# clevercool/ANT-Quantization

Hardware: AMD Instinct MI355X
Metric: Gelements/s quant-dequant + achieved HBM GB/s %peak, 4-bit ANT, 1/8 MI355X (higher is better)
Workload: dtype f32; 1 GPU; headline: 32 x [4096,4096] bf16 weight tensors per GPU, ANT 4-bit signed flint grid, calibrated per-row alpha, steady-state _forward; one step = ONE batched launch (antq_fakequant_batch) over all 32 tensors; io_dtype=bf16

## Files before the change

ant_quantization_amd/csrc/antq_host.h:

```cpp
#ifndef ANTQ_HOST_H
#define ANTQ_HOST_H

#include <hip/hip_runtime.h>
#include <stdint.h>
#include <string.h>

#include <algorithm>
#include <vector>

#include "../../include/antq.h"
#include "antq_internal.h"
#include "antq_device.h"
#include "antq_k_approx.h"

namespace antq {

extern thread_local int g_knob_u;
extern thread_local int g_knob_encwg;
extern thread_local int g_knob_x;
extern thread_local int g_knob_nearest_fast;
extern thread_local int g_knob_lane_rows;
extern thread_local int g_knob_a;
extern thread_local int g_knob_waves;
extern thread_local int g_knob_rot;
extern thread_local int g_knob_lane_u;
extern thread_local int g_knob_h;
extern thread_local int g_knob_hist;
extern thread_local int g_knob_sweep;
extern thread_local int g_knob_sort_short;
extern thread_local int g_knob_sort;
extern thread_local int g_knob_tk_group, g_knob_tk_blocks;
extern thread_local int g_knob_rows_stream;
extern thread_local int g_knob_hist_xmax;
extern thread_local int g_knob_exp;
extern thread_local int g_knob_schunks;
extern thread_local int g_knob_dlds;
extern thread_local int g_knob_hlds;

static inline bool plan_args_from_host(const void *plan_host, PlanArgs &pa)
{
    const PlanHeader *h = static_cast<const PlanHeader *>(plan_host);
    if (h->magic != kPlanMagic || h->version != kPlanVersion) return false;
    if (h->m < 1 || h->m > ANTQ_MAX_GRID || h->m_pad != ((h->m + 3) & ~3u)) return false;
    pa.kind = h->kind;
    pa.m = h->m;
    pa.m_pad = h->m_pad;
    pa.shift = h->shift;
    pa.kmin = h->kmin;
    pa.kmax = h->kmax;
    pa.keymask = h->keymask;
    pa.nbneg = h->nbneg;
    pa.fastlim = h->fastlim;
    pa.n_entries = (h->kind == kPlanLut) ? h->n_entries : 0;
    pa.tab_units = pa.n_entries + (pa.m_pad >> 2);
    pa.linear = h->linear;
    pa.lin_scale = h->lin_scale;
    pa.lin_bias = h->lin_bias;
    pa.adom = (h->kind == kPlanLut && g_knob_a != 0) ? h->adom : 0u;
    pa.xlim = h->xlim;
    pa.atab_slots = h->atab_slots;
    return true;
}

static inline const uint4 *plan_tab_ptr(const void *plan_dev)
{
    return reinterpret_cast<const uint4 *>(static_cast<const char *>(plan_dev) + sizeof(PlanHeader));
}

static inline size_t lds_table(const PlanArgs &pa, bool idx)
{
    const size_t plain = (size_t)pa.tab_units * 16;
    return pa.adom ? std::max(plain, (size_t)atab_units(pa.atab_slots, pa.m_pad, idx) * 16) : plain;
}

}

#endif
```

ant_quantization_amd/csrc/antq_kernels.hip:

```cpp
#include <type_traits>

#include "antq_host.h"
#include "antq_k_fakequant.h"
#include "antq_k_nearest.h"
#include "antq_k_aux.h"
#include "antq_k_reduce.h"
#include "antq_k_search.h"

namespace antq {

thread_local int g_knob_u = 0;
thread_local int g_knob_encwg = 2048;
thread_local int g_knob_x = 1;
thread_local int g_knob_nearest_fast = 1;
thread_local int g_knob_lane_rows = 1;
thread_local int g_knob_a = 1;
thread_local int g_knob_waves = 0;
thread_local int g_knob_lane_u = 0;
thread_local int g_knob_rot = 0;
thread_local int g_knob_h = 1;
thread_local int g_knob_hlds = -1;
thread_local int g_knob_dlds = -1;
thread_local int g_knob_schunks = 0;
thread_local int g_knob_exp = 0;
thread_local int g_knob_hist = 1;
thread_local int g_knob_hist_xmax = 1;
thread_local int g_knob_rows_stream = 1;
thread_local int g_knob_tk_group = 0;
thread_local int g_knob_tk_blocks = 0;
thread_local int g_knob_sort_short = 1;
thread_local int g_knob_sort = 1;
thread_local int g_knob_sweep = 1;

}

using namespace antq;

extern "C" int antq_abi_version(void) { return ANTQ_ABI_VERSION; }

extern "C" const char *antq_strerror(int code)
{
    switch (code) {
    case ANTQ_OK: return "ok";
    case ANTQ_ERR_ARG: return "invalid argument";
    case ANTQ_ERR_UNSUPPORTED: return "unsupported dtype / size for this entry point";
    case ANTQ_ERR_PLAN: return "malformed or undersized plan blob";
    case ANTQ_ERR_LAUNCH: return "HIP kernel launch failed";
    case ANTQ_ERR_ALIGN: return "pointer not aligned to the element size";
    default: return "unknown antq error";
    }
}

extern "C" int antq_nearest(const void *x, void *z, int16_t *idx, size_t n, const void *grid, int m, int dtype,
                            void *stream)
{
    if (n == 0) return ANTQ_OK;
    if (!x || !z || !grid || m < 1) return ANTQ_ERR_ARG;
    if (m > ANTQ_MAX_GRID) return ANTQ_ERR_UNSUPPORTED;
    hipStream_t st = static_cast<hipStream_t>(stream);
    if (dtype == ANTQ_F32 || dtype == ANTQ_F64) {
        const size_t blocks = (n + 1023) / 1024;
        if (blocks > 0x7fffffffull) return ANTQ_ERR_UNSUPPORTED;
        if (dtype == ANTQ_F32) {
            if (m <= 256 && g_knob_nearest_fast)
                hipLaunchKernelGGL((k_nearest_fast<float>), dim3((unsigned)((n + 2047) / 2048)), dim3(256), 0, st,
                                   static_cast<const float *>(x), static_cast<float *>(z), idx, n,
                                   static_cast<const float *>(grid), m);
            else
                hipLaunchKernelGGL((k_nearest<float>), dim3((unsigned)blocks), dim3(256), 0, st,
                                   static_cast<const float *>(x), static_cast<float *>(z), idx, n,
                                   static_cast<const float *>(grid), m);
        } else {
            if (m <= 256 && g_knob_nearest_fast)
                hipLaunchKernelGGL((k_nearest_fast<double>), dim3((unsigned)((n + 2047) / 2048)), dim3(256), 0, st,
                                   static_cast<const double *>(x), static_cast<double *>(z), idx, n,
                                   static_cast<const double *>(grid), m);
            else
                hipLaunchKernelGGL((k_nearest<double>), dim3((unsigned)blocks), dim3(256), 0, st,
                                   static_cast<const double *>(x), static_cast<double *>(z), idx, n,
                                   static_cast<const double *>(grid), m);
        }
    } else if (dtype == ANTQ_BF16 || dtype == ANTQ_F16) {
        const size_t blocks = (n + 255) / 256;
        if (blocks > 0x7fffffffull) return ANTQ_ERR_UNSUPPORTED;
        if (dtype == ANTQ_BF16)
            hipLaunchKernelGGL((k_nearest16<bf16_tag>), dim3((unsigned)blocks), dim3(256), 0, st, x, z, idx, n,
                               static_cast<const float *>(grid), m);
        else
            hipLaunchKernelGGL((k_nearest16<f16_tag>), dim3((unsigned)blocks), dim3(256), 0, st, x, z, idx, n,
                               static_cast<const float *>(grid), m);
    } else {
        return ANTQ_ERR_ARG;
    }
    return hipGetLastError() == hipSuccess ? ANTQ_OK : ANTQ_ERR_LAUNCH;
}

static int launch_nearest_plan(const void *x, void *z, int16_t *idx, size_t n, const void *plan_host, const void *plan_dev,
                               const float *gcheck, int m_check, int *stale, int dtype, void *stream)
{
    if (n == 0) return ANTQ_OK;
    if (!x || !z || !plan_host || !plan_dev) return ANTQ_ERR_ARG;
    PlanArgs pa;
    if (!plan_args_from_host(plan_host, pa)) return ANTQ_ERR_PLAN;
    if (gcheck && (uint32_t)m_check != pa.m) return ANTQ_ERR_ARG;
    const int epl = dtype == ANTQ_F32 ? 4 : (dtype == ANTQ_BF16 || dtype == ANTQ_F16) ? 8 : 0;
    if (!epl) return ANTQ_ERR_UNSUPPORTED;
    if (n % epl || reinterpret_cast<uintptr_t>(x) % 16 || reinterpret_cast<uintptr_t>(z) % 16 ||
        (idx && reinterpret_cast<uintptr_t>(idx) % 16))
        return ANTQ_ERR_UNSUPPORTED;
    const size_t n_vec = n / epl;
    hipStream_t st = static_cast<hipStream_t>(stream);
    const size_t lds = (size_t)pa.tab_units * 16;
    const bool u2 = !gcheck && lds <= 2048;
// ... 33 lines not shown
{
    if (!grid_dev || m < 1) return ANTQ_ERR_ARG;
    return launch_nearest_plan(x, z, idx, n, plan_host, plan_dev, grid_dev, m, stale, dtype, stream);
}

extern "C" int antq_affine(const float *x, float *out, int32_t *q, size_t rows, size_t row_len, int k,
                           const float *xmin, const float *xmax, int per_row, void *stream)
{
    if (rows == 0 || row_len == 0) return ANTQ_OK;
    if (!x || !out || !xmin || !xmax || k < 1 || k > 24) return ANTQ_ERR_ARG;
    const size_t n = rows * row_len;
    hipStream_t st = static_cast<hipStream_t>(stream);
    const bool vec = (per_row ? row_len : n) % 4 == 0 && reinterpret_cast<uintptr_t>(x) % 16 == 0 &&
                     reinterpret_cast<uintptr_t>(out) % 16 == 0 && (!q || reinterpret_cast<uintptr_t>(q) % 16 == 0);
    if (vec) {
        const size_t n_vec = n / 4, vpr = (per_row ? row_len : n) / 4;
        const size_t blocks = (n_vec + 256 * kAffineU - 1) / (256 * kAffineU);
        if (blocks > 0x7fffffffull) return ANTQ_ERR_UNSUPPORTED;
        hipLaunchKernelGGL(k_affine_vec, dim3((unsigned)blocks), dim3(256), 0, st, reinterpret_cast<const uint4 *>(x),
                           reinterpret_cast<uint4 *>(out), reinterpret_cast<int4 *>(q), n_vec, vpr, k, xmin, xmax,
                           per_row ? 1 : 0);
        return hipGetLastError() == hipSuccess ? ANTQ_OK : ANTQ_ERR_LAUNCH;
    }
    const size_t blocks = (n + 255) / 256;
    if (blocks > 0x7fffffffull) return ANTQ_ERR_UNSUPPORTED;
    hipLaunchKernelGGL(k_affine, dim3((unsigned)blocks), dim3(256), 0, st, x, out, q, n,
                       row_len, k, xmin, xmax, per_row ? 1 : 0);
    return hipGetLastError() == hipSuccess ? ANTQ_OK : ANTQ_ERR_LAUNCH;
}

extern "C" int antq_copy(const void *src, void *dst, size_t bytes, void *stream)
{
    if (bytes == 0) return ANTQ_OK;
    if (!src || !dst || bytes % 16 || reinterpret_cast<uintptr_t>(src) % 16 || reinterpret_cast<uintptr_t>(dst) % 16)
        return ANTQ_ERR_ARG;
    const size_t n_vec = bytes / 16;
    const size_t blocks = (n_vec + 1023) / 1024;
    if (blocks > 0x7fffffffull) return ANTQ_ERR_UNSUPPORTED;
    hipLaunchKernelGGL(k_copy, dim3((unsigned)blocks), dim3(256), 0, static_cast<hipStream_t>(stream),
                       static_cast<const uint4 *>(src), static_cast<uint4 *>(dst), n_vec);
    return hipGetLastError() == hipSuccess ? ANTQ_OK : ANTQ_ERR_LAUNCH;
}

namespace antq {
int prefetch_unit_fq();
int prefetch_unit_batch();
int prefetch_unit_search();
}
extern "C" int antq_prefetch_kernels(void)
{
    hipFuncAttributes at;
    int rc = hipFuncGetAttributes(&at, reinterpret_cast<const void *>(&k_copy)) == hipSuccess ? ANTQ_OK : ANTQ_ERR_LAUNCH;
    if (antq::prefetch_unit_fq() != ANTQ_OK) rc = ANTQ_ERR_LAUNCH;
    if (antq::prefetch_unit_batch() != ANTQ_OK) rc = ANTQ_ERR_LAUNCH;
    if (antq::prefetch_unit_search() != ANTQ_OK) rc = ANTQ_ERR_LAUNCH;
    (void)hipGetLastError();
    return rc;
}

extern "C" int antq_debug_set(int key, int value)
{
    if (key == 0) g_knob_u = value;
    else if (key == 1) g_knob_encwg = value > 0 ? value : 2048;
    else if (key == 2) g_knob_x = value;
    else if (key == 3) g_knob_nearest_fast = value;
    else if (key == 4) g_knob_a = value;
    else if (key == 5) g_knob_lane_rows = value;
    else if (key == 6) g_knob_waves = value;
    else if (key == 7) g_knob_lane_u = value;
    else if (key == 8) g_knob_rot = value;
    else if (key == 9) g_knob_h = value;
    else if (key == 10) g_knob_hlds = value;
    else if (key == 11) g_knob_dlds = value;
    else if (key == 12) g_knob_schunks = value;
    else if (key == 13) g_knob_exp = value;
    else if (key == 14) g_knob_hist = value;
    else if (key == 15) g_knob_hist_xmax = value;
    else if (key == 16) g_knob_rows_stream = value;
    else if (key == 17) g_knob_tk_group = value;
    else if (key == 18) g_knob_tk_blocks = value;
    else if (key == 19) g_knob_sweep = value;
    else if (key == 20) g_knob_sort = value;
    else if (key == 21) g_knob_sort_short = value;
    else return ANTQ_ERR_ARG;
    return ANTQ_OK;
}

namespace antq {

template <typename T>
static int launch_absmax(const void *x, float *amax, size_t rows, size_t row_len, int per_row, hipStream_t st, bool zero = true)
{
    constexpr int EPL = IO<T>::EPL;
    const bool al = reinterpret_cast<uintptr_t>(x) % 16 == 0;
    const int vec_ok = per_row ? (al && row_len % EPL == 0) : al;
    if (per_row && vec_ok) {
        const size_t vpr = row_len / EPL;
        if (vpr <= 64 && (vpr & (vpr - 1)) == 0) {
            int vshift = 0;
            while (((size_t)1 << vshift) < vpr) vshift++;
            const size_t n_vec = rows * vpr, gblocks = (n_vec + 1023) / 1024;
            if (gblocks > 0x7fffffffull) return ANTQ_ERR_UNSUPPORTED;
            hipLaunchKernelGGL((k_absmax_groups<T>), dim3((unsigned)gblocks), dim3(256), 0, st, static_cast<const uint4 *>(x), amax,
                               n_vec, (uint32_t)vpr, vshift);
            return hipGetLastError() == hipSuccess ? ANTQ_OK : ANTQ_ERR_LAUNCH;
        }
    }
    if (per_row && vec_ok && g_knob_rows_stream && rows <= 0x7fffffffull) {
        const size_t vpr = row_len / EPL;
        const dim3 g((unsigned)(rows < 262144u ? rows : 262144u)), b(64);
        const uint4 *xv = static_cast<const uint4 *>(x);
        bool done = true;
        if (vpr == 128) hipLaunchKernelGGL((k_absmax_rows<T, 2>), g, b, 0, st, xv, amax, (uint32_t)rows);
        else if (vpr == 256) hipLaunchKernelGGL((k_absmax_rows<T, 4>), g, b, 0, st, xv, amax, (uint32_t)rows);
        else if (vpr == 512) hipLaunchKernelGGL((k_absmax_rows<T, 8>), g, b, 0, st, xv, amax, (uint32_t)rows);
        else if (vpr == 1024) hipLaunchKernelGGL((k_absmax_rows<T, 16>), g, b, 0, st, xv, amax, (uint32_t)rows);
        else done = false;
        if (done) return hipGetLastError() == hipSuccess ? ANTQ_OK : ANTQ_ERR_LAUNCH;
    }
    size_t waves = per_row ? rows : (rows * row_len + 64 * EPL * 4 - 1) / (64 * EPL * 4);
    size_t blocks = (waves + 3) / 4;
    if (blocks > (per_row ? 4096u : 256u)) blocks = per_row ? 4096 : 256;
    if (blocks < 1) blocks = 1;
    if (!per_row && zero) hipLaunchKernelGGL(k_zero_f32, dim3(1), dim3(64), 0, st, amax);
    hipLaunchKernelGGL((k_absmax<T>), dim3((unsigned)blocks), dim3(256), 0, st, x, amax, rows, row_len, per_row, vec_ok);
    return hipGetLastError() == hipSuccess ? ANTQ_OK : ANTQ_ERR_LAUNCH;
}
}

namespace antq {
template <typename T>
static int launch_alpha_grad(const void *x, const void *out, const void *gout, double *gsum, double *ws, size_t rows,
                             size_t row_len, int per_row, hipStream_t st)
{
    static_assert(kPartialStride == kPtCand, "k_sum_partials reads partials kPtCand doubles apart");
    constexpr int EPL = IO<T>::EPL;
    const bool al = (reinterpret_cast<uintptr_t>(x) | reinterpret_cast<uintptr_t>(out) | reinterpret_cast<uintptr_t>(gout)) % 16 == 0;
    const int vec_ok = per_row ? (al && row_len % EPL == 0) : al;
    size_t waves = per_row ? rows : (rows * row_len + 64 * EPL * 2 - 1) / (64 * EPL * 2);
    size_t blocks = (waves + 3) / 4;
    const size_t cap = per_row ? 4096 : 1024;
    if (blocks > cap) blocks = cap;
    if (blocks < 1) blocks = 1;
    hipLaunchKernelGGL((k_alpha_grad<T>), dim3((unsigned)blocks), dim3(256), 0, st, x, out, gout, gsum, ws, rows, row_len,
                       per_row, vec_ok);
    if (!per_row) hipLaunchKernelGGL(k_sum_partials, dim3(1), dim3(256), 0, st, ws, (uint32_t)blocks, 1, gsum);
    return hipGetLastError() == hipSuccess ? ANTQ_OK : ANTQ_ERR_LAUNCH;
}
}

extern "C" int antq_alpha_grad(const void *x, const void *out, const void *gout, size_t rows, size_t row_len, int per_row,
                               double *gsum, void *workspace, int dtype, void *stream)
{
    if (rows == 0 || row_len == 0) return ANTQ_OK;
    if (!x || !out || !gout || !gsum || (!per_row && !workspace)) return ANTQ_ERR_ARG;
    double *ws = static_cast<double *>(workspace);
    hipStream_t st = static_cast<hipStream_t>(stream);
    switch (dtype) {
    case ANTQ_F32: return launch_alpha_grad<float>(x, out, gout, gsum, ws, rows, row_len, per_row ? 1 : 0, st);
    case ANTQ_BF16: return launch_alpha_grad<bf16_tag>(x, out, gout, gsum, ws, rows, row_len, per_row ? 1 : 0, st);
    case ANTQ_F16: return launch_alpha_grad<f16_tag>(x, out, gout, gsum, ws, rows, row_len, per_row ? 1 : 0, st);
    default: return ANTQ_ERR_UNSUPPORTED;
    }
}

namespace antq {
// ... 197 lines not shown
```

ant_quantization_amd/csrc/antq_search.hip:

```cpp
#include <cstdio>
#include <cstdlib>
#include <mutex>
#include <vector>

#include "antq_host.h"
#include "antq_k_fakequant.h"
#include "antq_k_search.h"
#include "antq_k_hist.h"
#include "antq_k_sweep.h"
#include "antq_k_sortsearch.h"

#include <type_traits>

namespace antq {

constexpr unsigned kSearchMinVpr = 64;

template <typename T>
static bool hist_eligible(size_t n, bool ovp, const void *x, int nflat)
{
    if constexpr (std::is_same<T, float>::value) return false;
    if (g_knob_hist == 0 || (ovp && g_knob_hist == 3) || n % 8 != 0 || n >= ((size_t)1 << 31) || reinterpret_cast<uintptr_t>(x) % 16 != 0) return false;
    if (g_knob_hist == 2) return true;
    if (ovp) return n >= ((size_t)1 << 20) && (double)n * (double)nflat >= 1.5e8;
    return n >= ((size_t)1 << 19);
}
static bool hist_outlier_bound(const void *plan_host, float gmax, float &bound)
{
    const PlanHeader *h = static_cast<const PlanHeader *>(plan_host);
    if (h->kind != kPlanLut || !h->hdom || !(gmax > 0.0f)) return false;
    const HThr *tl = plan_tlist(plan_host);
    float tmin = INFINITY;
    for (uint32_t i = 0; i < h->h_nthr; i++) {
        const bool lo_out = (tl[i].flags & 1u) != 0u, hi_out = (tl[i].flags & 2u) != 0u;
        if (lo_out != hi_out) tmin = std::min(tmin, fabsf(tl[i].T));
    }
    if (!(tmin < INFINITY)) tmin = 3.0e38f;
    bound = tmin / gmax * 0.999f;
    return true;
}
struct HistXmax {
    float *out = nullptr;
    bool taken = false;
};

template <typename T>
static int launch_hist_search(const void *x, size_t n, const float *xmax, const float *ratios, int ncand, const HistTypes &ht,
                              double *sse, void *ws, bool pairs, float tmin_over_gmax, const int **run_if, hipStream_t st,
                              HistXmax *hx = nullptr)
{
    if constexpr (std::is_same<T, float>::value) {
        return ANTQ_ERR_UNSUPPORTED;
    } else {
        const size_t nv = n / 8;
        uint32_t G = (uint32_t)std::min<size_t>(std::max<size_t>(n / 65536, 16), (size_t)kHistMaxG);
        G = (G + 7u) & ~7u;
        char *w = static_cast<char *>(ws);
        uint32_t *slabs = reinterpret_cast<uint32_t *>(w);
        uint32_t *count = reinterpret_cast<uint32_t *>(w + kHistCountOff);
        HistPairs hp;
        hp.xmax = xmax; hp.ratios = ratios; hp.ncand = ncand; hp.tmin_over_gmax = tmin_over_gmax;
        hp.seg = reinterpret_cast<uint32_t *>(w + kHistSegOff);
        hp.seg_count = reinterpret_cast<uint32_t *>(w + kHistSegCountOff);
        hp.flags = reinterpret_cast<int *>(w + kHistFlagsOff);
        hp.list = reinterpret_cast<uint32_t *>(w + kHistListOff);
        const unsigned nflat = (unsigned)(ht.ntypes * ncand);
        size_t lds = 0;
        for (int t = 0; t < ht.ntypes; t++) lds = std::max(lds, (size_t)ht.pa[t].tab_units * 16);
        if (pairs) {
            hipLaunchKernelGGL(k_hist_clear_flags, dim3(1), dim3(64), 0, st, hp.flags);
            hipLaunchKernelGGL((k_hist16<T, true>), dim3(2 * G), dim3(1024), 0, st, static_cast<const uint4 *>(x), nv, G, slabs, hp, nullptr);
            hipLaunchKernelGGL((k_hist_reduce<true>), dim3(256), dim3(256), 0, st, slabs, G, count, hp, G * 16u);
            hipLaunchKernelGGL((k_hist_score<T, true>), dim3(nflat), dim3(1024), lds, st, count, xmax, ratios, ncand, ht, sse, hp);
            *run_if = hp.flags;
        } else {
            float *const xo = (hx && !hx->taken) ? hx->out : nullptr;
            if (hx && xo) hx->taken = true;
            if (xo)
                hipLaunchKernelGGL((k_hist16<T, false, true>), dim3(2 * G), dim3(1024), 0, st, static_cast<const uint4 *>(x), nv, G, slabs, hp, xo);
            else
                hipLaunchKernelGGL((k_hist16<T, false>), dim3(2 * G), dim3(1024), 0, st, static_cast<const uint4 *>(x), nv, G, slabs, hp, nullptr);
            hipLaunchKernelGGL((k_hist_reduce<false>), dim3(256), dim3(256), 0, st, slabs, G, count, hp, 0u);
            hipLaunchKernelGGL((k_hist_score<T, false>), dim3(nflat), dim3(1024), lds, st, count, xmax, ratios, ncand, ht, sse, hp);
        }
        return hipGetLastError() == hipSuccess ? ANTQ_OK : ANTQ_ERR_LAUNCH;
    }
}

struct SearchGrid {
    size_t blocks;
    int chunks, chunk;
};
template <typename K>
// ... 141 lines not shown
    const size_t nv = n / EPL;
    const size_t ws_bytes = antq_search_workspace_bytes();
    size_t G = std::min<size_t>((nv + 255) / 256, 2048);
    const uint32_t per_group = 64;
    G = std::min(G, ws_bytes / ((size_t)cells_max * 8) - (2048 / per_group + 2));
    if (G < 16) return ANTQ_ERR_UNSUPPORTED;
    const uint32_t ngroups = (uint32_t)((G + per_group - 1) / per_group);
    int lg = 0;
    while (((size_t)1 << lg) < n) lg++;
    const int fbits = std::min(38, 53 - lg);
    long long *slabs = static_cast<long long *>(ws);
    for (int t = 0; t < ntypes; t++) {
        const uint32_t ncells = sweep_slab_cells(ty[t].n_thr, cp), nint = 2u * ty[t].n_thr * cp + 132u;
        long long *part = slabs + G * (size_t)ncells, *tot = part + (size_t)ngroups * ncells;
        const size_t lds = sweep_lds_bytes(ty[t].n_thr, cp);
        hipLaunchKernelGGL((k_search_sweep<T, OVP, true>), dim3((unsigned)G), dim3(64), lds, st, static_cast<const uint4 *>(x), nv, (size_t)1,
                           xmax, ratios, sse + (size_t)t * ncand, ty[t], (uint32_t)ncand, cp, slabs, fbits);
        hipLaunchKernelGGL(k_sweep_pt_total, dim3((ncells + 255) / 256, ngroups), dim3(256), 0, st, slabs, (uint32_t)G, per_group, ncells, nint, part);
        hipLaunchKernelGGL(k_sweep_pt_total, dim3((ncells + 255) / 256, 1), dim3(256), 0, st, part, ngroups, ngroups, ncells, nint, tot);
        hipLaunchKernelGGL(k_sweep_pt_finish, dim3(1), dim3(64), lds, st, tot, xmax, ratios, sse + (size_t)t * ncand, ty[t], (uint32_t)ncand, cp, fbits);
    }
    return hipGetLastError() == hipSuccess ? ANTQ_OK : ANTQ_ERR_LAUNCH;
}


constexpr uint32_t kSortLdsMax = 64 * 1024;
static bool sort_type_ok(const void *plan_host, float gmax)
{
    const PlanHeader *ph = static_cast<const PlanHeader *>(plan_host);
    return ph->kind == kPlanLut && ph->hdom && ph->h_nthr > 0 && ph->h_nthr <= 64u && gmax > 0.0f;
}
static bool sort_fill_types(SortTypes &stt, int ntypes, const float *gmax, const void *const *plan_host, const void *const *plan_dev)
{
    memset(&stt, 0, sizeof(stt));
    if (ntypes < 1 || ntypes > kMaxTypes) return false;
    stt.ntypes = ntypes;
    uint32_t nmax = 0;
    for (int t = 0; t < ntypes; t++) {
        if (!sort_type_ok(plan_host[t], gmax[t])) return false;
        const PlanHeader *ph = static_cast<const PlanHeader *>(plan_host[t]);
        const HThr *tl = plan_tlist(plan_host[t]);
        SweepType &ty = stt.ty[t];
        ty.tlist = reinterpret_cast<const uint4 *>(static_cast<const char *>(plan_dev[t]) + ph->tlist_off);
        ty.grid = reinterpret_cast<const float *>(plan_tab_ptr(plan_dev[t]));
        ty.n_thr = ph->h_nthr;
        ty.m = ph->m;
        ty.gmax = gmax[t];
        const float flim = ph->fastlim * 0.99999f;
        ty.lim = flim < ph->xlim ? flim : ph->xlim;
        ty.kout_pos = ty.kout_neg = -1;
        stt.nneg[t] = 0;
        for (uint32_t k = 0; k < ph->h_nthr; k++) {
            const bool lo_out = (tl[k].flags & 1u) != 0u, hi_out = (tl[k].flags & 2u) != 0u;
            if (k > 0 && !(tl[k].T > tl[k - 1].T)) return false;
            if (tl[k].T < 0.0f) stt.nneg[t] = k + 1u;
            if (!lo_out && hi_out) { if (ty.kout_pos >= 0 || !(tl[k].T > 0.0f)) return false; ty.kout_pos = (int)k; }
            if (lo_out && !hi_out) { if (ty.kout_neg >= 0 || !(tl[k].T < 0.0f)) return false; ty.kout_neg = (int)k; }
        }
        nmax = std::max(nmax, ph->h_nthr);
    }
    stt.nthr_pad = (nmax + (uint32_t)kSortKS - 1u) / (uint32_t)kSortKS * (uint32_t)kSortKS;
    return true;
}
static int sort_piece(const SortTypes &stt, int ncand, bool ovp)
{
    const uint32_t nkg = stt.nthr_pad / (uint32_t)kSortKS;
    auto fits = [&](int nc) {
        const uint32_t ntc = (uint32_t)(stt.ntypes * nc);
        return sort_lds(ntc, stt.nthr_pad, stt.ntypes, ovp).total <= kSortLdsMax && ntc * nkg <= (uint32_t)(kSortNI * kSortNT) &&
               ntc <= (uint32_t)(kSortNL * kSortNT) && (!ovp || 4u * ntc <= (uint32_t)(kSortNC * kSortNT));
    };
    int nc = ncand;
    while (nc > 0 && !fits(nc)) nc = nc > 1 ? (nc + 1) / 2 : 0;
    return nc;
}
template <typename T, bool OVP>
static bool sort_shape_ok(const void *x, size_t rows, size_t row_len, int ncand, int ntypes)
{
    constexpr int EPL = IO<T>::EPL;
    if (!g_knob_sort || rows < 2 || ncand < 1 || ntypes < 1 || ntypes > kMaxTypes) return false;
    if (reinterpret_cast<uintptr_t>(x) % 16 != 0 || row_len % EPL != 0 || row_len < (g_knob_sort == 2 ? 128u : (OVP ? 256u : 128u))) return false;
    return !(OVP && (row_len & 1));
}
template <typename T, bool OVP>
static int launch_sorted(const void *x, size_t rows, size_t row_len, const float *xmax, const float *ratios, int ncand, int ntypes,
                         const float *gmax, const void *const *plan_host, const void *const *plan_dev, double *sse, hipStream_t st)
{
    constexpr int EPL = IO<T>::EPL;
    if (!sort_shape_ok<T, OVP>(x, rows, row_len, ncand, ntypes)) return ANTQ_ERR_UNSUPPORTED;
    SortTypes stt;
    if (!sort_fill_types(stt, ntypes, gmax, plan_host, plan_dev)) return ANTQ_ERR_UNSUPPORTED;
    {
        if (row_len <= (size_t)kSortKSh && g_knob_sort_short) {
            int piece = ncand;
            auto lds_of = [&](int nc) { return (((uint32_t)ntypes * kSortTy * 4u + 15u) & ~15u) + 4u * sort_short_wave_bytes((uint32_t)(ntypes * nc)); };
            while (piece > 1 && (lds_of(piece) > kSortLdsMax || ntypes * piece > 512)) piece = (piece + 1) / 2;
            const unsigned blocks = (unsigned)std::min<size_t>((rows + 3) / 4, (size_t)1 << 20);
            for (int c0 = 0; c0 < ncand; c0 += piece) {
                const int nc = std::min(piece, ncand - c0);
                hipLaunchKernelGGL((k_search_sorted_short<T, OVP>), dim3(blocks), dim3(256), lds_of(nc), st, static_cast<const uint4 *>(x),
                                   (uint32_t)(row_len / EPL), rows, xmax, ratios + c0, sse + (size_t)c0 * rows, stt, (uint32_t)nc, (uint32_t)ncand);
            }
            return hipGetLastError() == hipSuccess ? ANTQ_OK : ANTQ_ERR_LAUNCH;
        }
    }
    const int piece = sort_piece(stt, ncand, OVP);
    if (piece < 1) return ANTQ_ERR_UNSUPPORTED;
    const unsigned blocks = (unsigned)std::min<size_t>(rows, (size_t)1 << 20);
    for (int c0 = 0; c0 < ncand; c0 += piece) {
        const int nc = std::min(piece, ncand - c0);
        const SortLds L = sort_lds((uint32_t)(ntypes * nc), stt.nthr_pad, ntypes, OVP);
        hipLaunchKernelGGL((k_search_sorted<T, OVP, false>), dim3(blocks), dim3(kSortNT), L.total, st, static_cast<const uint4 *>(x),
                           row_len / EPL, rows, xmax, ratios + c0, sse + (size_t)c0 * rows, stt, (uint32_t)nc, (uint32_t)ncand, nullptr);
    }
    return hipGetLastError() == hipSuccess ? ANTQ_OK : ANTQ_ERR_LAUNCH;
}

template <typename T>
static bool sort_pt_shape_ok(const void *x, size_t n, int ncand)
{
    constexpr int EPL = IO<T>::EPL;
    if (!g_knob_sort || sizeof(T) != 4 || ncand < 1) return false;
    return reinterpret_cast<uintptr_t>(x) % 16 == 0 && n % EPL == 0 && n >= (g_knob_sort == 2 ? 4096u : (1u << 20)) && n < ((size_t)1 << 40);
}
template <typename T, bool OVP>
static int launch_sorted_pt(const void *x, size_t n, const float *xmax, const float *ratios, int ncand, int ntypes, const float *gmax,
                            const void *const *plan_host, const void *const *plan_dev, double *sse, void *ws, hipStream_t st)
{
    constexpr int EPL = IO<T>::EPL;
    if (!sort_pt_shape_ok<T>(x, n, ncand) || !ws || (OVP && (n & 1))) return ANTQ_ERR_UNSUPPORTED;
    SortTypes stt;
    if (!sort_fill_types(stt, ntypes, gmax, plan_host, plan_dev)) return ANTQ_ERR_UNSUPPORTED;
    const int piece = sort_piece(stt, ncand, OVP);
    if (piece < 1) return ANTQ_ERR_UNSUPPORTED;
    const size_t nv = n / EPL, nchunks = (n + kSortK - 1) / kSortK;
    const uint32_t nkg = stt.nthr_pad / (uint32_t)kSortKS, per_group = 32;
    const size_t ws_cells = antq_search_workspace_bytes() / 8;
    double *slabs = static_cast<double *>(ws);
    for (int c0 = 0; c0 < ncand; c0 += piece) {
        const int nc = std::min(piece, ncand - c0);
        const uint32_t ntc = (uint32_t)(ntypes * nc), ncell = ntc * nkg + ntc + (OVP ? 4u * ntc : 0u) + 1u;
        size_t G = std::min<size_t>((nchunks + 2) / 3, 768);
        G = std::min(G, ws_cells / ncell - (768 / per_group + 2));
        if (G < 1 || ws_cells / ncell < 768 / per_group + 3) return ANTQ_ERR_UNSUPPORTED;
        const uint32_t ngroups = (uint32_t)((G + per_group - 1) / per_group);
        double *part = slabs + G * (size_t)ncell, *tot = part + (size_t)ngroups * ncell;
        const SortLds L = sort_lds(ntc, stt.nthr_pad, ntypes, OVP);
        hipLaunchKernelGGL((k_search_sorted<T, OVP, true>), dim3((unsigned)G), dim3(kSortNT), L.total, st, static_cast<const uint4 *>(x), nv,
                           (size_t)1, xmax, ratios + c0, sse + c0, stt, (uint32_t)nc, (uint32_t)ncand, slabs);
        hipLaunchKernelGGL(k_sort_pt_total, dim3((ncell + 255) / 256, ngroups), dim3(256), 0, st, slabs, (uint32_t)G, per_group, ncell, part);
        hipLaunchKernelGGL(k_sort_pt_total, dim3((ncell + 255) / 256, 1), dim3(256), 0, st, part, ngroups, ngroups, ncell, tot);
        hipLaunchKernelGGL(k_sort_pt_finish, dim3((ntc + 255) / 256), dim3(256), 0, st, tot, ntc, nkg, OVP ? 1 : 0, (uint32_t)nc, (uint32_t)ncand, sse + c0);
    }
    return hipGetLastError() == hipSuccess ? ANTQ_OK : ANTQ_ERR_LAUNCH;
}

template <typename T, bool OVP>
static int launch_search(const void *x, size_t rows, size_t row_len, const float *xmax, int per_row,
                         const float *ratios, int ncand, float gmax, const PlanArgs &pa, const void *plan_host,
                         const void *plan_dev, double *sse, double *ws, hipStream_t st, HistXmax *hx = nullptr)
{
    constexpr int EPL = IO<T>::EPL;
    const size_t lds = (size_t)pa.tab_units * 16;
    if (reinterpret_cast<uintptr_t>(x) % 16 != 0 || (per_row ? row_len : rows * row_len) % EPL != 0) {
        size_t strips = per_row ? rows : (rows * row_len + 16383) / 16384;
        size_t blocks = (strips + 3) / 4;
        const size_t ychunks = ((size_t)ncand + kPtCand - 1) / kPtCand;
        if (blocks > 256 * 8) blocks = 256 * 8;
        if (!per_row) {
            if (ychunks > (size_t)kWsSlots) return ANTQ_ERR_UNSUPPORTED;
            blocks = std::min(blocks, (size_t)kWsSlots / ychunks);
        }
        hipLaunchKernelGGL((k_search_sse_scalar<T, OVP>), dim3((unsigned)blocks, (unsigned)ychunks), dim3(256), lds, st, x, rows,
                           row_len, xmax, per_row, ratios, ncand, gmax, sse, ws, pa, plan_tab_ptr(plan_dev));
        if (!per_row)
            hipLaunchKernelGGL(k_sum_partials, dim3((unsigned)ncand), dim3(256), 0, st, ws, (uint32_t)blocks, kPtCand, sse);
        return hipGetLastError() == hipSuccess ? ANTQ_OK : ANTQ_ERR_LAUNCH;
    }
    if (per_row && rows > 1) {
        const void *ph1[1] = {plan_host}, *pd1[1] = {plan_dev};
        int rc = launch_sorted<T, OVP>(x, rows, row_len, xmax, ratios, ncand, 1, &gmax, ph1, pd1, sse, st);
        if (rc != ANTQ_ERR_UNSUPPORTED) return rc;
        rc = launch_sweep<T, OVP>(x, rows, row_len, xmax, ratios, ncand, 1, &gmax, ph1, pd1, sse, st);
        if (rc != ANTQ_ERR_UNSUPPORTED) return rc;
    }
    if (!per_row) { row_len = rows * row_len; rows = 1; }
    const int *run_if = nullptr;
    float bound = 0.0f;
    if (rows == 1 && hist_eligible<T>(row_len, OVP, x, ncand) && (!OVP || hist_outlier_bound(plan_host, gmax, bound))) {
        HistTypes ht;
        memset(&ht, 0, sizeof(ht));
// ... 479 lines not shown
```

Before: 1644 Gelem/s.

## Add binned-histogram search kernel for bf16 rows in sorted calibration search

Adds a new k_search_bins kernel that replaces per-row sorting with a histogram over bf16 high-16-bit key bins for the calibration alpha search. Elements inside a central band are accumulated directly, the rest are counted into bins, and per-threshold SSE is derived from the bin prefix sums. It is meant to avoid the cost of sorting each row during the per-row alpha search. The measured headline is the steady-state fake-quant launch, so this calibration-path change probably does not touch the timed region. It also brings a lot of new numerics-sensitive code.

```diff
diff --git a/ant_quantization_amd/csrc/antq_host.h b/ant_quantization_amd/csrc/antq_host.h
--- a/ant_quantization_amd/csrc/antq_host.h
+++ b/ant_quantization_amd/csrc/antq_host.h
@@ -28,6 +28,7 @@
 extern thread_local int g_knob_hist;
 extern thread_local int g_knob_sweep;
 extern thread_local int g_knob_sort_short;
+extern thread_local int g_knob_bins;
 extern thread_local int g_knob_sort;
 extern thread_local int g_knob_tk_group, g_knob_tk_blocks;
 extern thread_local int g_knob_rows_stream;
diff --git a/ant_quantization_amd/csrc/antq_k_binsearch.h b/ant_quantization_amd/csrc/antq_k_binsearch.h
--- /dev/null
+++ b/ant_quantization_amd/csrc/antq_k_binsearch.h
@@ -0,0 +1,506 @@
+#ifndef ANTQ_K_BINSEARCH_H
+#define ANTQ_K_BINSEARCH_H
+
+#include "antq_k_sortsearch.h"
+
+namespace antq {
+
+__host__ __device__ inline uint32_t bin_ceil16(uint32_t K)
+{
+    const uint32_t h = K >> 16;
+    const uint32_t kh = (h << 16) | (h < 0x8000u ? 0xffffu : 0u);
+    return h + (kh >= K ? 0u : 1u);
+}
+__device__ __forceinline__ float bin_value(uint32_t h) { return sort_unkey((h << 16) | (h < 0x8000u ? 0xffffu : 0u)); }
+
+struct BinLds {
+    uint32_t off_c, off_x, off_s, off_v, off_misc, total;
+};
+__host__ __device__ inline BinLds bin_lds(uint32_t nbin, uint32_t ntc, uint32_t nthr_pad, int ntypes, bool ovp)
+{
+    BinLds L;
+    const uint32_t nitems = ntc * (nthr_pad / (uint32_t)kSortKS);
+    uint32_t o = (uint32_t)kSortPad * 4u;
+    o = o > (nbin / 2u + 2u) * 8u ? o : (nbin / 2u + 2u) * 8u;
+    const uint32_t fin = (nitems + (ovp ? 4u * ntc : 0u)) * 8u;
+    o = o > fin ? o : fin;
+    o = (o + 15u) & ~15u;
+    L.off_c = o;     o += (nbin + 2u) * 4u;
+    o = (o + 15u) & ~15u;
+    L.off_x = o;     o += sort_inline(ovp) ? ntc * 2u * 4u : ntc * nthr_pad * 4u;
+    L.off_s = o;     o += ntc * 4u;
+    o = (o + 15u) & ~15u;
+    L.off_v = o;     o += (uint32_t)ntypes * kSortTy * 4u;
+    o = (o + 15u) & ~15u;
+    L.off_misc = o;  o += 512u;
+    L.total = o;
+    return L;
+}
+
+template <typename T, bool OVP>
+__global__ void __launch_bounds__(kSortNT, 3)
+k_search_bins(const uint4 *__restrict__ x, size_t vpr, size_t rows, const float *__restrict__ xmax, const float *__restrict__ ratios,
+              double *__restrict__ sse, SortTypes st, uint32_t ncand, uint32_t ncand_all, uint32_t nbin)
+{
+    static_assert(std::is_same<T, bf16_tag>::value, "the bin table holds bf16 values");
+    constexpr int EPL = IO<T>::EPL;
+    constexpr int VPT = kSortEPT / EPL;
+    constexpr size_t VPC = kSortK / EPL;
+    extern __shared__ __attribute__((aligned(16))) uint4 smem[];
+    const uint32_t tid = threadIdx.x, lane = tid & 63u, wave = tid >> 6;
+    const uint32_t ntypes = (uint32_t)st.ntypes, ntc = ntypes * ncand, nthr_pad = st.nthr_pad, nkg = nthr_pad / (uint32_t)kSortKS;
+    const uint32_t nitems = ntc * nkg;
+    auto type_of = [&](uint32_t tc) { return (tc >= ncand ? 1u : 0u) + (tc >= 2u * ncand ? 1u : 0u) + (tc >= 3u * ncand ? 1u : 0u); };
+    const BinLds L = bin_lds(nbin, ntc, nthr_pad, st.ntypes, OVP);
+    char *base = reinterpret_cast<char *>(smem);
+    uint32_t *sK = reinterpret_cast<uint32_t *>(base);
+    long long *sPB = reinterpret_cast<long long *>(base);
+    uint32_t *sC = reinterpret_cast<uint32_t *>(base + L.off_c);
+    uint32_t *sX = reinterpret_cast<uint32_t *>(base + L.off_x);
+    float *sS = reinterpret_cast<float *>(base + L.off_s);
+    float *sV = reinterpret_cast<float *>(base + L.off_v);
+    unsigned long long *sScan = reinterpret_cast<unsigned long long *>(base + L.off_misc);
+    double *sScanD = reinterpret_cast<double *>(base + L.off_misc + 128);
+    int *sFlag = reinterpret_cast<int *>(base + L.off_misc + 192);
+    uint32_t *sBand = reinterpret_cast<uint32_t *>(base + L.off_misc + 256);
+    uint32_t *sCC = reinterpret_cast<uint32_t *>(base + L.off_misc + 288);
+    long long *sCS = reinterpret_cast<long long *>(base + L.off_misc + 304);
+    uint32_t *sWC = reinterpret_cast<uint32_t *>(base + L.off_misc + 336);
+    long long *sWS = reinterpret_cast<long long *>(base + L.off_misc + 352);
+
+#pragma unroll
+    for (int t = 0; t < kMaxTypes; t++)
+        if (t < st.ntypes) sort_fill_type(sV + (uint32_t)t * kSortTy, st.ty[t], st.nneg[t], tid);
+    __syncthreads();
+    auto ty_nthr = [&](uint32_t t) { return reinterpret_cast<const uint32_t *>(sV + t * kSortTy)[130]; };
+    auto ty_kpos = [&](uint32_t t) { return (int)reinterpret_cast<const uint32_t *>(sV + t * kSortTy)[131]; };
+    auto ty_kneg = [&](uint32_t t) { return (int)reinterpret_cast<const uint32_t *>(sV + t * kSortTy)[132]; };
+    auto ty_gmax = [&](uint32_t t) { return sV[t * kSortTy + 133u]; };
+    auto ty_lim = [&](uint32_t t) { return sV[t * kSortTy + 134u]; };
+    auto ty_nneg = [&](uint32_t t) { return reinterpret_cast<const uint32_t *>(sV + t * kSortTy)[136]; };
+    auto ty_m = [&](uint32_t t) { return (int)reinterpret_cast<const uint32_t *>(sV + t * kSortTy)[135]; };
+    auto ty_grid = [&](uint32_t t) {
+        const float *g = st.ty[0].grid;
+#pragma unroll
+        for (int u = 1; u < kMaxTypes; u++) g = (uint32_t)u == t ? st.ty[u].grid : g;
+        return g;
+    };
+
+    const size_t nchunks_row = (vpr + VPC - 1) / VPC;
+    for (size_t row = blockIdx.x; row < rows; row += gridDim.x) {
+        const float xm = xmax[row];
+        const uint4 *xr = x + row * vpr;
+        if (xm == 0.0f || xm != xm) {
+            for (uint32_t tc = tid; tc < ntc; tc += kSortNT) {
+                const uint32_t t = type_of(tc), c = tc - t * ncand;
+                sse[((size_t)t * ncand_all + c) * rows + row] = __builtin_nan("");
+            }
+            continue;
+        }
+        bool ok = true;
+        for (uint32_t tc = tid; tc < ntc; tc += kSortNT) {
+            const uint32_t t = type_of(tc), c = tc - t * ncand;
+            const Scale sc = make_scale(xm * ratios[c], ty_gmax(t));
+            sS[tc] = sc.s;
+            ok = ok && sc.ok && (sc.s > 0.0f);
+        }
+        __syncthreads();
+        for (uint32_t tc = tid; tc < ntc; tc += kSortNT) {
+            const uint32_t t = type_of(tc), c = tc - t * ncand;
+            if (c > 0u) ok = ok && (sS[tc] >= sS[tc - 1u]);
+        }
+        if (tid == 0u) *sFlag = 0;
+        __syncthreads();
+        if (!ok) atomicOr(sFlag, 1);
+        __syncthreads();
+        const bool usable = *sFlag == 0;
+        constexpr bool INL = sort_inline(OVP);
+        if constexpr (INL) {
+            for (uint32_t tc = tid; tc < ntc; tc += kSortNT) {
+                const uint32_t t = type_of(tc);
+                const float *v = sV + t * kSortTy;
+                const double sd = (double)sS[tc];
+                sX[2u * tc] = (usable && ty_kpos(t) >= 0) ? sort_threshold_key(v, (uint32_t)ty_kpos(t), sd) : kSortSent;
+                sX[2u * tc + 1u] = (usable && ty_kneg(t) >= 0) ? sort_threshold_key(v, (uint32_t)ty_kneg(t), sd) : 0u;
+            }
+        }
+        const uint32_t q_thr = kSortNT / nthr_pad, r_thr = kSortNT - q_thr * nthr_pad;
+        for (uint32_t p = tid, tc = tid / nthr_pad, k = tid - (tid / nthr_pad) * nthr_pad; !INL && p < ntc * nthr_pad; p += kSortNT) {
+            const uint32_t t = type_of(tc);
+            uint32_t key = kSortSent;
+            if (usable && k < ty_nthr(t)) {
+                key = sort_threshold_key(sV + t * kSortTy, k, (double)sS[tc]);
+            }
+            sX[p] = key;
+            k += r_thr;
+            tc += q_thr + (k >= nthr_pad ? 1u : 0u);
+            k -= k >= nthr_pad ? nthr_pad : 0u;
+        }
+        double acc[kSortNI], corr[kSortNC], lit[kSortNL];
+#pragma unroll
+        for (int u = 0; u < kSortNI; u++) acc[u] = 0.0;
+#pragma unroll
+        for (int u = 0; u < kSortNC; u++) corr[u] = 0.0;
+#pragma unroll
+        for (int u = 0; u < kSortNL; u++) lit[u] = 0.0;
+        int ex = 0;
+        (void)frexpf(xm, &ex);
+        const double F = __builtin_ldexp(1.0, 38 - ex), unit = __builtin_ldexp(1.0, ex - 38);
+        float Lx = 0.0f;
+        if (usable) {
+            Lx = __builtin_ldexpf(0.999f, ex + 8);
+            for (uint32_t t = 0; t < ntypes; t++) Lx = fminf(Lx, ty_lim(t) * sS[t * ncand] * 0.999f);
+        }
+        {
+            uint32_t hlo = 0u, hhi = 0x10000u;
+            const uint32_t t = tid >> 6, k = tid & 63u;
+            if (usable && t < ntypes && k < ty_nthr(t)) {
+                const uint32_t h = bin_ceil16(sort_threshold_key(sV + t * kSortTy, k, (double)sS[t * ncand]));
+                if (h <= 0x8000u) hlo = h; else hhi = h;
+            }
+#pragma unroll
+            for (int off = 32; off >= 1; off >>= 1) {
+                hlo = max(hlo, (uint32_t)__shfl_xor((int)hlo, off, 64));
+                hhi = min(hhi, (uint32_t)__shfl_xor((int)hhi, off, 64));
+            }
+            if (lane == 0u) { sBand[wave] = hlo; sBand[4u + wave] = hhi; }
+        }
+        for (uint32_t i = tid; i < nbin + 2u; i += kSortNT) sC[i] = 0u;
+        __syncthreads();
+        uint32_t cLo = 0u, cHi = 0x10000u;
+#pragma unroll
+        for (uint32_t w = 0; w < kSortNT / 64; w++) { cLo = max(cLo, sBand[w]); cHi = min(cHi, sBand[4u + w]); }
+        uint32_t kNlo = sort_key(-Lx) >> 16, kPhi = (sort_key(Lx) >> 16) + 1u;
+        uint32_t nN = cLo > kNlo ? cLo - kNlo : 0u, nP = kPhi > cHi ? kPhi - cHi : 0u;
+        if (nN + nP + 2u > nbin) {
+            const uint32_t capN = (nbin - 2u) / 2u, capP = nbin - 2u - capN;
+            if (nN > capN) { kNlo = cLo - capN; nN = capN; Lx = fminf(Lx, -bin_value(kNlo)); }
+            if (nP > capP) { kPhi = cHi + capP; nP = capP; Lx = fminf(Lx, bin_value(kPhi)); }
+        }
+        const uint32_t o = (nN & 1u) ? 0u : 1u, zc = o + nN, nrow = zc + 1u + nP;
+        auto bin_key = [&](uint32_t i) { return i < zc ? kNlo + i - o : cHi + (i - zc - 1u); };
+        float XoP = __builtin_inff(), XoN = -__builtin_inff();
+        if (OVP && usable) {
+            for (uint32_t t = 0; t < ntypes; t++) {
+                if (INL) {
+                    if (ty_kpos(t) >= 0) XoP = fminf(XoP, sort_unkey(sX[2u * (t * ncand)]));
+                    if (ty_kneg(t) >= 0) XoN = fmaxf(XoN, sort_unkey(sX[2u * (t * ncand) + 1u]));
+                } else {
+                    if (ty_kpos(t) >= 0) XoP = fminf(XoP, sort_unkey(sX[(t * ncand) * nthr_pad + (uint32_t)ty_kpos(t)]));
+                    if (ty_kneg(t) >= 0) XoN = fmaxf(XoN, sort_unkey(sX[(t * ncand) * nthr_pad + (uint32_t)ty_kneg(t)]));
+                }
+            }
+        }
+        double Q = 0.0;
+        uint32_t nch_done = 0, Kreg = 0;
+        uint32_t cC = 0;
+        long long cS = 0;
+
+        for (size_t ch = 0; ch < nchunks_row; ch++) {
+            float xs[kSortEPT];
+            uint32_t nreg = 0, nlit = 0, ncap = 0;
+            uint32_t litmask = 0, capmask = 0;
+#pragma unroll
+            for (int j = 0; j < VPT; j++) {
+                const size_t vi = ch * VPC + (size_t)j * kSortNT + tid;
+                const bool live = vi < vpr;
+                float xf[EPL];
+                {
+                    const uint4 v = live ? xr[vi] : make_uint4(0u, 0u, 0u, 0u);
+                    IO<T>::unpack(v, xf);
+                }
+#pragma unroll
+                for (int e = 0; e < EPL; e += 2) {
+                    const int r = j * EPL + e;
+                    const float a = xf[e], b = xf[e + 1];
+                    bool la = live && !(fabsf(a) < Lx), lb = live && !(fabsf(b) < Lx);
+                    bool cap = false;
+                    if (OVP) {
+                        la = lb = (la || lb);
+                        cap = live && !la && ((a >= XoP) || (a < XoN) || (b >= XoP) || (b < XoN));
+                    }
+                    const bool ra = live && !la, rb = live && !lb;
+                    xs[r] = a;
+                    xs[r + 1] = b;
+                    Q = __builtin_fma((double)(ra ? a : 0.0f), (double)(ra ? a : 0.0f), Q);
+                    Q = __builtin_fma((double)(rb ? b : 0.0f), (double)(rb ? b : 0.0f), Q);
+                    nreg += (ra ? 1u : 0u) + (rb ? 1u : 0u);
+                    nlit += (la ? 1u : 0u) + (lb ? 1u : 0u);
+                    litmask |= (la ? 1u : 0u) << r | (lb ? 1u : 0u) << (r + 1);
+                    if (OVP && cap) { ncap++; capmask |= 1u << r; }
+#pragma unroll
+                    for (int h2 = 0; h2 < 2; h2++) {
+                        const float xv = h2 ? b : a;
+                        if (!(h2 ? rb : ra)) continue;
+                        const uint32_t kh = sort_key(xv) >> 16;
+                        if (kh >= cLo && kh < cHi) {
+                            cC++;
+                            cS += sweep_fixed(xv, F);
+                        } else {
+                            const uint32_t bi = kh < cLo ? o + (kh - kNlo) : zc + 1u + (kh - cHi);
+                            atomicAdd(&sC[min(bi, nbin)], 1u);
+                        }
+                    }
+                }
+            }
+            unsigned long long pk = (unsigned long long)nreg | (unsigned long long)nlit << 16 | (unsigned long long)ncap << 32, inc = pk;
+#pragma unroll
+            for (int off = 1; off < 64; off <<= 1) {
+                const unsigned long long tv = (unsigned long long)__shfl_up((long long)inc, off, 64);
+                if (lane >= (uint32_t)off) inc += tv;
+            }
+            const uint32_t par = (nch_done & 1u) * 4u;
+            nch_done++;
+            if (lane == 63u) sScan[par + wave] = inc;
+            __syncthreads();
+            unsigned long long before = 0, total = 0;
+#pragma unroll
+            for (uint32_t w = 0; w < kSortNT / 64; w++) {
+                const unsigned long long v = sScan[par + w];
+                before += w < wave ? v : 0ull;
+                total += v;
+            }
+            Kreg += (uint32_t)(total & 0xffffu);
+            const uint32_t tot_lit = (uint32_t)((total >> 16) & 0xffffu), tot_cap = (uint32_t)((total >> 32) & 0xffffu);
+            if (tot_lit | tot_cap) {
+                const unsigned long long excl = before + inc - pk;
+                uint32_t pl = (uint32_t)((excl >> 16) & 0xffffu), pc = (uint32_t)((excl >> 32) & 0xffffu);
+                float *sList = reinterpret_cast<float *>(sK);
+#pragma unroll
+                for (int r = 0; r < kSortEPT; r++)
+                    if ((litmask >> r) & 1u) sList[pl++] = xs[r];
+                if (OVP) {
+#pragma unroll
+                    for (int r = 0; r < kSortEPT; r += 2)
+                        if ((capmask >> r) & 1u) {
+                            sK[kSortK - 2u - 2u * pc] = sort_key(xs[r]);
+                            sK[kSortK - 1u - 2u * pc] = sort_key(xs[r + 1]);
+                            pc++;
+                        }
+                }
+                __syncthreads();
+                if (tot_lit) {
+                    for (uint32_t tc = tid, ui = 0; tc < ntc; tc += kSortNT, ui++) {
+                        const uint32_t t = type_of(tc);
+                        const float *grid = ty_grid(t);
+                        const int gm = ty_m(t);
+                        const float s = sS[tc], lim = usable ? ty_lim(t) : 0.0f;
+                        const uint32_t *X = sX + (INL ? 0u : tc * nthr_pad);
+                        const float *v = sV + t * kSortTy;
+                        const uint32_t nthr_t = ty_nthr(t);
+                        auto q_of = [&](float xv, float &d, bool &tab) -> float {
+                            d = xv / s;
+                            tab = fabsf(d) < lim;
+                            if (tab) {
+                                const uint32_t kx = sort_key(xv);
+                                uint32_t lo = 0, hi = nthr_t;
+                                while (lo < hi) {
+                                    const uint32_t mid = (lo + hi) >> 1;
+                                    if (INL ? d >= v[66u + mid] : kx >= X[mid]) lo = mid + 1u; else hi = mid;
+                                }
+                                return v[lo];
+                            }
+                            return sort_literal_q(xv, s, v, grid, gm, d);
+                        };
+                        auto term_of = [&](float q, float d, bool tab, float xv) -> double {
+                            if (tab) {
+                                const double e = (double)(q * s) - (double)xv;
+                                return e * e;
+                            }
+                            return sweep_term(q, d, s, xv);
+                        };
+                        double sum_l = 0.0;
+                        for (uint32_t i = 0; i < tot_lit; i += OVP ? 2u : 1u) {
+                            const float xa_ = sList[i];
+                            float da, db = 0.0f;
+                            bool ta, tb = false;
+                            float qa = q_of(xa_, da, ta), qb = 0.0f;
+                            if (OVP) {
+                                const float xb_ = sList[i + 1u];
+                                qb = q_of(xb_, db, tb);
+                                const bool me = fabsf(qa) > 32.0f, mo = fabsf(qb) > 32.0f;
+                                const bool ve = mo && !me;
+                                qa = qa * (ve ? 0.0f : 1.0f);
+                                qb = qb * (me ? 0.0f : 1.0f);
+                                sum_l += term_of(qb, db, tb, xb_);
+                            }
+                            sum_l += term_of(qa, da, ta, xa_);
+                        }
+#pragma unroll
+                        for (int u = 0; u < kSortNL; u++) lit[u] += (uint32_t)u == ui ? sum_l : 0.0;
+                    }
+                }
+                if (OVP && tot_cap) {
+                    for (uint32_t it = tid, ui = 0; it < 4u * ntc; it += kSortNT, ui++) {
+                        const uint32_t tc = it >> 2, j0 = it & 3u, t = type_of(tc);
+                        const uint32_t *X = sX + (INL ? 0u : tc * nthr_pad);
+                        const float s = sS[tc];
+                        const float *v = sV + t * kSortTy;
+                        const uint32_t nthr_t = ty_nthr(t);
+                        const uint32_t kp = INL ? sX[2u * tc] : (ty_kpos(t) >= 0 ? X[ty_kpos(t)] : kSortSent);
+                        const uint32_t kn = INL ? sX[2u * tc + 1u] : (ty_kneg(t) >= 0 ? X[ty_kneg(t)] : 0u);
+                        double sum_c = 0.0;
+                        for (uint32_t i = j0; i < tot_cap; i += 4u) {
+                            const uint32_t ka = sK[kSortK - 2u - 2u * i], kb = sK[kSortK - 1u - 2u * i];
+                            const bool me = ka >= kp || ka < kn, mo = kb >= kp || kb < kn;
+                            if (me || mo) {
+                                const uint32_t kv = me ? kb : ka;
+                                const float vv = sort_unkey(kv);
+                                const float dvv = vv / s;
+                                uint32_t lo = 0, hi = nthr_t;
+                                while (lo < hi) {
+                                    const uint32_t mid = (lo + hi) >> 1;
+                                    if (INL ? dvv >= v[66u + mid] : kv >= X[mid]) lo = mid + 1u; else hi = mid;
+                                }
+                                const double O = (double)(v[lo] * s), dv = (double)vv;
+                                sum_c += dv * dv - (O - dv) * (O - dv);
+                            }
+                        }
+#pragma unroll
+                        for (int u = 0; u < kSortNC; u++) corr[u] += (uint32_t)u == ui ? sum_c : 0.0;
+                    }
+                }
+                __syncthreads();
+            }
+        }
+        if (Kreg != 0u) {
+#pragma unroll
+            for (int off = 32; off >= 1; off >>= 1) {
+                cC += (uint32_t)__shfl_xor((int)cC, off, 64);
+                cS += __shfl_xor(cS, off, 64);
+            }
+            if (lane == 0u) { sCC[wave] = cC; sCS[wave] = cS; }
+            __syncthreads();
+            uint32_t nc = 0;
+            long long sc = 0;
+#pragma unroll
+            for (uint32_t w = 0; w < kSortNT / 64; w++) { nc += sCC[w]; sc += sCS[w]; }
+            const uint32_t per = (nrow + kSortNT - 1u) / kSortNT, b0 = min(tid * per, nrow), b1 = min(b0 + per, nrow);
+            auto bin_cs = [&](uint32_t i, uint32_t &c, long long &s) {
+                if (i == zc) { c = nc; s = sc; return; }
+                c = sC[i];
+                s = c ? (long long)c * sweep_fixed(bin_value(bin_key(i)), F) : 0ll;
+            };
+            uint32_t mc = 0;
+            long long ms = 0;
+            for (uint32_t i = b0; i < b1; i++) {
+                uint32_t c;
+                long long s;
+                bin_cs(i, c, s);
+                mc += c;
+                ms += s;
+            }
+            uint32_t ic = mc;
+            long long is = ms;
+#pragma unroll
+            for (int off = 1; off < 64; off <<= 1) {
+                const uint32_t tc_ = (uint32_t)__shfl_up((int)ic, off, 64);
+                const long long ts_ = __shfl_up(is, off, 64);
+                if (lane >= (uint32_t)off) { ic += tc_; is += ts_; }
+            }
+            if (lane == 63u) { sWC[wave] = ic; sWS[wave] = is; }
+            __syncthreads();
+            uint32_t pc = ic - mc;
+            long long ps = is - ms;
+#pragma unroll
+            for (uint32_t w = 0; w < kSortNT / 64; w++) {
+                pc += w < wave ? sWC[w] : 0u;
+                ps += w < wave ? sWS[w] : 0ll;
+            }
+            for (uint32_t i = b0; i < b1; i++) {
+                uint32_t c;
+                long long s;
+                bin_cs(i, c, s);
+                sC[i] = pc;
+                if (!(i & 1u)) sPB[i >> 1] = ps;
+                pc += c;
+                ps += s;
+            }
+            long long Stot_i = 0;
+#pragma unroll
+            for (uint32_t w = 0; w < kSortNT / 64; w++) Stot_i += sWS[w];
+            if (tid == kSortNT - 1u) {
+                sC[nrow] = Kreg;
+                if (!(nrow & 1u)) sPB[nrow >> 1] = Stot_i;
+            }
+            __syncthreads();
+            const double Stot = (double)Stot_i * unit, dn = (double)Kreg;
+            const uint32_t q_it = kSortNT / nkg, r_it = kSortNT - q_it * nkg;
+            for (uint32_t it = tid, ui = 0, tc = tid / nkg, kg = tid - (tid / nkg) * nkg; it < nitems; it += kSortNT, ui++) {
+                const uint32_t t = type_of(tc);
+                const float s = sS[tc];
+                const float *v = sV + t * kSortTy + kg * (uint32_t)kSortKS;
+                const uint32_t *X = sX + (INL ? 0u : tc * nthr_pad + kg * (uint32_t)kSortKS);
+                uint32_t bi[kSortKS];
+#pragma unroll
+                for (int j = 0; j < kSortKS; j++) {
+                    uint32_t Xk;
+                    if constexpr (INL) {
+                        const uint32_t kk = kg * (uint32_t)kSortKS + (uint32_t)j;
+                        Xk = (usable && kk < ty_nthr(t)) ? sort_threshold_key(sV + t * kSortTy, kk, (double)s) : kSortSent;
+                    } else {
+                        Xk = X[j];
+                    }
+                    const uint32_t h = bin_ceil16(Xk);
+                    bi[j] = h < cHi ? o + min(h > kNlo ? h - kNlo : 0u, nN) : zc + 1u + min(h - cHi, nP);
+                }
+                const uint32_t nb = ty_nneg(t);
+                double part = 0.0;
+                if (kg == 0u) {
+                    const double Ob_ = (double)(sV[t * kSortTy + nb] * s);
+                    part = dn * Ob_ * Ob_ - 2.0 * Ob_ * Stot;
+                }
+#pragma unroll
+                for (int j = 0; j < kSortKS; j++) {
+                    const uint32_t i = bi[j], p = sC[i];
+                    long long slt = sPB[i >> 1];
+                    if (i & 1u) slt += (long long)(p - sC[i - 1u]) * sweep_fixed(bin_value(bin_key(i - 1u)), F);
+                    const bool below = kg * (uint32_t)kSortKS + (uint32_t)j < nb;
+                    const double N = below ? -(double)p : (double)(Kreg - p);
+                    const double S = (double)(below ? -slt : Stot_i - slt) * unit;
+                    const double Oa = (double)(v[j] * s), Ob = (double)(v[j + 1] * s);
+                    part += (Ob - Oa) * ((Ob + Oa) * N - 2.0 * S);
+                }
+#pragma unroll
+                for (int u = 0; u < kSortNI; u++) acc[u] += (uint32_t)u == ui ? part : 0.0;
+                kg += r_it;
+                tc += q_it + (kg >= nkg ? 1u : 0u);
+                kg -= kg >= nkg ? nkg : 0u;
+            }
+        }
+#pragma unroll
+        for (int off = 32; off >= 1; off >>= 1) Q += __shfl_xor(Q, off, 64);
+        __syncthreads();
+        if (lane == 0u) sScanD[wave] = Q;
+        __syncthreads();
+        double Qw = 0.0;
+#pragma unroll
+        for (uint32_t w = 0; w < kSortNT / 64; w++) Qw += sScanD[w];
+        double *fA = reinterpret_cast<double *>(base), *fC = fA + nitems;
+#pragma unroll
+        for (int u = 0; u < kSortNI; u++)
+            if (tid + (uint32_t)u * kSortNT < nitems) fA[tid + (uint32_t)u * kSortNT] = acc[u];
+        if (OVP) {
+#pragma unroll
+            for (int u = 0; u < kSortNC; u++)
+                if (tid + (uint32_t)u * kSortNT < 4u * ntc) fC[tid + (uint32_t)u * kSortNT] = corr[u];
+        }
+        __syncthreads();
+        for (uint32_t tc = tid, ui = 0; tc < ntc; tc += kSortNT, ui++) {
+            double sum = Qw;
+            for (uint32_t kg = 0; kg < nkg; kg++) sum += fA[tc * nkg + kg];
+            double l = 0.0;
+#pragma unroll
+            for (int u = 0; u < kSortNL; u++) l = (uint32_t)u == ui ? lit[u] : l;
+            sum += l;
+            if (OVP) sum += (fC[4u * tc] + fC[4u * tc + 1u]) + (fC[4u * tc + 2u] + fC[4u * tc + 3u]);
+            const uint32_t t = type_of(tc), c = tc - t * ncand;
+            sse[((size_t)t * ncand_all + c) * rows + row] = sum;
+        }
+        __syncthreads();
+    }
+}
+
+}
+
+#endif
diff --git a/ant_quantization_amd/csrc/antq_kernels.hip b/ant_quantization_amd/csrc/antq_kernels.hip
--- a/ant_quantization_amd/csrc/antq_kernels.hip
+++ b/ant_quantization_amd/csrc/antq_kernels.hip
@@ -29,6 +29,7 @@
 thread_local int g_knob_tk_group = 0;
 thread_local int g_knob_tk_blocks = 0;
 thread_local int g_knob_sort_short = 1;
+thread_local int g_knob_bins = 1;
 thread_local int g_knob_sort = 1;
 thread_local int g_knob_sweep = 1;
 
@@ -228,6 +229,7 @@
     else if (key == 19) g_knob_sweep = value;
     else if (key == 20) g_knob_sort = value;
     else if (key == 21) g_knob_sort_short = value;
+    else if (key == 22) g_knob_bins = value;
     else return ANTQ_ERR_ARG;
     return ANTQ_OK;
 }
diff --git a/ant_quantization_amd/csrc/antq_search.hip b/ant_quantization_amd/csrc/antq_search.hip
--- a/ant_quantization_amd/csrc/antq_search.hip
+++ b/ant_quantization_amd/csrc/antq_search.hip
@@ -1,3 +1,4 @@
+#include <cmath>
 #include <cstdio>
 #include <cstdlib>
 #include <mutex>
@@ -9,6 +10,7 @@
 #include "antq_k_hist.h"
 #include "antq_k_sweep.h"
 #include "antq_k_sortsearch.h"
+#include "antq_k_binsearch.h"
 
 #include <type_traits>
 
@@ -316,6 +318,59 @@
     if (reinterpret_cast<uintptr_t>(x) % 16 != 0 || row_len % EPL != 0 || row_len < (g_knob_sort == 2 ? 128u : (OVP ? 256u : 128u))) return false;
     return !(OVP && (row_len & 1));
 }
+constexpr uint32_t kBinLdsMax = 160u * 1024u / 3u & ~255u;
+template <typename T>
+static bool bin_shape_ok(size_t row_len)
+{
+    if (!std::is_same<T, bf16_tag>::value || !g_knob_bins || row_len > 65536u) return false;
+    return g_knob_bins == 2 || row_len > (size_t)kSortKSh;
+}
+static uint32_t bin_count(const SortTypes &stt, const void *const *plan_host)
+{
+    double limg = HUGE_VAL, posg = HUGE_VAL, negg = HUGE_VAL;
+    for (int t = 0; t < stt.ntypes; t++) {
+        const double gm = (double)stt.ty[t].gmax;
+        limg = std::min(limg, (double)stt.ty[t].lim / gm);
+        const HThr *tl = plan_tlist(plan_host[t]);
+        for (uint32_t k = 0; k < stt.ty[t].n_thr; k++) {
+            const double M = 0.5 * ((double)std::nextafter(tl[k].T, -HUGE_VALF) + (double)tl[k].T);
+            if (M > 0.0) posg = std::min(posg, M / gm);
+            else negg = std::min(negg, -M / gm);
+        }
+    }
+    if (!(limg > 0.0) || !(limg < HUGE_VAL)) return 0;
+    auto side = [&](double m) -> uint64_t {
+        if (m == HUGE_VAL) return 0;
+        const double R = limg / m * (1.0 + 1e-5);
+        if (!(R < 1e12)) return (uint64_t)1 << 40;
+        return 128u * (uint64_t)((R > 1.0 ? (int)std::floor(std::log2(R)) : 0) + 2) + 2u;
+    };
+    const uint64_t n = side(posg) + side(negg) + 2u;
+    return n < ((uint64_t)1 << 20) ? (uint32_t)n : 0u;
+}
+template <typename T, bool OVP>
+struct BinLaunch {
+    static int run(const void *, size_t, size_t, const float *, const float *, int, int, const void *const *, double *, hipStream_t,
+                   const SortTypes &, int) { return ANTQ_ERR_UNSUPPORTED; }
+};
+template <bool OVP>
+struct BinLaunch<bf16_tag, OVP> {
+    static int run(const void *x, size_t rows, size_t row_len, const float *xmax, const float *ratios, int ncand, int ntypes,
+                   const void *const *plan_host, double *sse, hipStream_t st, const SortTypes &stt, int piece)
+    {
+        constexpr int EPL = IO<bf16_tag>::EPL;
+        const uint32_t nbin = bin_shape_ok<bf16_tag>(row_len) ? bin_count(stt, plan_host) : 0u;
+        if (!nbin || bin_lds(nbin, (uint32_t)(ntypes * piece), stt.nthr_pad, ntypes, OVP).total > kBinLdsMax) return ANTQ_ERR_UNSUPPORTED;
+        const unsigned blocks = (unsigned)std::min<size_t>(rows, (size_t)1 << 20);
+        for (int c0 = 0; c0 < ncand; c0 += piece) {
+            const int nc = std::min(piece, ncand - c0);
+            const BinLds L = bin_lds(nbin, (uint32_t)(ntypes * nc), stt.nthr_pad, ntypes, OVP);
+            hipLaunchKernelGGL((k_search_bins<bf16_tag, OVP>), dim3(blocks), dim3(kSortNT), L.total, st, static_cast<const uint4 *>(x),
+                               row_len / EPL, rows, xmax, ratios + c0, sse + (size_t)c0 * rows, stt, (uint32_t)nc, (uint32_t)ncand, nbin);
+        }
+        return ANTQ_OK;
+    }
+};
 template <typename T, bool OVP>
 static int launch_sorted(const void *x, size_t rows, size_t row_len, const float *xmax, const float *ratios, int ncand, int ntypes,
                          const float *gmax, const void *const *plan_host, const void *const *plan_dev, double *sse, hipStream_t st)
@@ -341,6 +396,8 @@
     const int piece = sort_piece(stt, ncand, OVP);
     if (piece < 1) return ANTQ_ERR_UNSUPPORTED;
     const unsigned blocks = (unsigned)std::min<size_t>(rows, (size_t)1 << 20);
+    if (BinLaunch<T, OVP>::run(x, rows, row_len, xmax, ratios, ncand, ntypes, plan_host, sse, st, stt, piece) == ANTQ_OK)
+        return hipGetLastError() == hipSuccess ? ANTQ_OK : ANTQ_ERR_LAUNCH;
     for (int c0 = 0; c0 < ncand; c0 += piece) {
         const int nc = std::min(piece, ncand - c0);
         const SortLds L = sort_lds((uint32_t)(ntypes * nc), stt.nthr_pad, ntypes, OVP);
```

After: 1645 Gelem/s, median of 6. About the same (+0.0%).
